# weihaoysgs/ssvio

Measured on AMD Instinct MI355X. Metric: stereo frames/s (ORB extract + row-band match + triangulate + one local BA per frame) on 1241x376, higher is better.
Workload: dtype u8 (front-end) + f64 (BA)

## Files before the change

include/ssx_test_hooks.h:

```cpp
#ifndef SSX_TEST_HOOKS_H
#define SSX_TEST_HOOKS_H
#include "ssx.h"

#ifdef __cplusplus
extern "C" {
#endif

SSX_API int32_t ssx_ba_window_selftest(uint32_t seed, int32_t steps);

SSX_API int64_t ssx_debug_kernel_dynamic_lds(const char* kernel);
SSX_API void ssx_debug_set_dense_slabs(int32_t mode);

SSX_API void ssx_debug_set_trial_finish(int32_t mode);

SSX_API double ssx_ba_debug_prepare_seconds(const ssx_ba_problem* prob, int32_t reps);

SSX_API int32_t ssx_ba_debug_upload_format(const ssx_ba_problem* prob);

SSX_API uint64_t ssx_ba_debug_prepare_digest(const ssx_ba_problem* prob, int32_t threads);

typedef struct ssx_orb_plan_info {
  int32_t status, n_buffers;
  uint64_t digest[3];
  uint64_t arena_bytes, buf_off[32], buf_bytes[32];
  int32_t nlevels, out_cap;
  int32_t lvl_rows[8], lvl_cols[8], feat[8], lvl_cell0[9], gauss_tile0[9];
  char error[256];
} ssx_orb_plan_info;
SSX_API ssx_status ssx_orb_debug_plan(int32_t rows, int32_t cols, int32_t images, const ssx_orb_params* prm, int32_t has_mask,
                                      int32_t detect_only, int32_t unchecked, ssx_orb_plan_info* out);


SSX_API ssx_status ssx_ba_linearize(ssx_ctx* ctx, const ssx_ba_problem* prob, double huber_delta, int32_t jac_mode,
                            double* Hpp, double* bp, double* Hll, double* bl, double* Hpl, double* err,
                            double* chi2);

SSX_API ssx_status ssx_orb_stage_level(ssx_ctx* ctx, int32_t image, int32_t level, int32_t blurred,
                                       uint8_t* out, int32_t out_cap, int32_t* rows, int32_t* cols);
SSX_API ssx_status ssx_orb_stage_candidates(ssx_ctx* ctx, int32_t image, int32_t level, int32_t cap,
                                            ssx_keypoint* out, int32_t* n);

SSX_API ssx_status ssx_lk_stage_level(ssx_ctx* ctx, int32_t which, int32_t level, uint8_t* out, int32_t out_cap,
                                      int32_t* rows, int32_t* cols);
SSX_API ssx_status ssx_lk_stage_deriv(ssx_ctx* ctx, int32_t level, int16_t* out, int32_t out_cap, int32_t* rows,
                                      int32_t* cols);

enum { SSX_LK_STAGED = 0, SSX_LK_ARENA = 1, SSX_LK_EACH = 2, SSX_LK_IN_PLACE = 3 };
enum { SSX_LK_K_PYRAMID = 0, SSX_LK_K_PAD_LEVEL0 = 1, SSX_LK_K_PYR_DOWN = 2, SSX_LK_K_SCHARR = 3, SSX_LK_K_TRACK = 4 };
enum { SSX_LK_SPANS = 7, SSX_LK_MAX_LAUNCHES = 32, SSX_LK_MAX_INFO_JOBS = 256 };
typedef struct ssx_lk_call_info {
  int32_t status;
  char error[256];
  int32_t levels, win, pad, rows[8], cols[8], pitch[8];
  uint64_t off[8], doff[8], pyr_bytes, deriv_words;
  int32_t fused_ok, use_fused, scharr_now, intake;
  uint64_t span_off[7], span_bytes[7], in_bytes, host_end, io_bytes, arena_bytes;
  int32_t n_launches, n_jobs;
  struct { int32_t kernel, grid[3], which, level; } launch[32];
  uint8_t slot_flags[256], job_roles[256];
} ssx_lk_call_info;
typedef struct ssx_lk_job_facts {
  int32_t slot, fresh, n, prev_stride, next_stride, reserved;
  int64_t next_off;
// ... 25 lines not shown
```

ssvio_amd/csrc/orb.hip:

```cpp
#include <algorithm>
#include <cfloat>
#include <cmath>
#include <vector>

#include "ctx.hpp"
#include "orb_ws.hpp"
#include "../../include/ssx_test_hooks.h"

namespace ssxorb {

__constant__ __attribute__((aligned(16))) int8_t c_pattern[256 * 4] = {
#include "brief_pattern.inc"
};
__constant__ int c_umax[16] = {15, 15, 15, 15, 14, 14, 14, 13, 13, 12, 11, 10, 9, 8, 6, 3};
__constant__ int c_gauss[7] = {18, 34, 49, 55, 49, 34, 18};
__constant__ int c_ring_dx[16] = {0, 1, 2, 3, 3, 3, 2, 1, 0, -1, -2, -3, -3, -3, -2, -1};
__constant__ int c_ring_dy[16] = {3, 3, 2, 1, 0, -1, -2, -3, -3, -3, -2, -1, 0, 1, 2, 3};

struct ResizeQuad {
  uint32_t s0;
  uint32_t sel0, sel1;
  uint32_t pad;
  uint32_t w[4];
};
// ... 405 lines not shown

__device__ __forceinline__ bool gauss_tile_at_edge(int rows, int cols, int x0)
{
  return rows >= 8 && cols >= 8 && (x0 == 0 || x0 + GT_W + 4 > cols);
}
__device__ __forceinline__ void gauss_fix_edges(uint8_t* sIn, int cols, int x0, int t)
{
  if (t < 6 * (GT_H + 6)) {
    const int r = t / 6, k = t - 6 * r;
    const int x = k < 3 ? k - 3 : cols + k - 3;
    const int xs = k < 3 ? -x : 2 * cols - 2 - x;
    const int b = x - x0 + 4, bs = xs - x0 + 4;
    if (b >= 0 && b < GT_PITCH && bs >= 0 && bs < GT_PITCH) sIn[r * GT_PITCH + b] = sIn[r * GT_PITCH + bs];
  }
}

__global__ __launch_bounds__(256) void k_gauss7(OrbDev o)
{
  __shared__ __attribute__((aligned(16))) uint8_t sIn[(GT_H + 6) * GT_PITCH];
  __shared__ __attribute__((aligned(16))) uint32_t sRowP[(GT_H + 6) / 2 * GT_W];
  static_assert((GT_H + 6) % 2 == 0, "rows are processed in pairs");
  const int img = blockIdx.y, t = threadIdx.x;
  int level = 0;
  while (level + 1 < o.nlevels && (int)blockIdx.x >= o.gauss_tile0[level + 1]) ++level;
  const int grp = blockIdx.x - o.gauss_tile0[level];
  const int rows = o.lvl_rows[level], cols = o.lvl_cols[level], pitch = o.lvl_pitch[level];
  const int tiles_x = (cols + GT_W - 1) / GT_W;
  const int run = o.gauss_run;
  const int groups_x = (tiles_x + run - 1) / run;
  const int ty_ = grp / groups_x, tx0 = (grp - ty_ * groups_x) * run;
  const int tx1 = min(tx0 + run, tiles_x);
  const int y0 = ty_ * GT_H;
  const uint8_t* src = o.pyr + (size_t)img * o.pyr_bytes + o.lvl_off[level];
  uint8_t* dst = o.blur + (size_t)img * o.pyr_bytes + o.lvl_off[level];
  constexpr int NDW = GT_PITCH / 4;
  uint32_t ld[GT_NLD];
  gauss_load_tile(src, rows, cols, pitch, tx0 * GT_W, y0, t, ld);
  uint32_t outv[4];
  const int og = t & 31, orq = t >> 5;
  auto store_tile = [&](int x0s) {
    const int x = x0s + 4 * og;
#pragma unroll
    for (int j = 0; j < 4; ++j) {
      const int y = y0 + 4 * orq + j;
      if (y < rows && x < pitch) *reinterpret_cast<uint32_t*>(dst + (size_t)y * pitch + x) = outv[j];
    }
  };
#pragma unroll 1
  for (int tx_ = tx0; tx_ < tx1; ++tx_) {
  const int x0 = tx_ * GT_W;
  if (tx_ > tx0) __syncthreads();
#pragma unroll
  for (int k = 0; k < GT_NLD; ++k) {
    const int i = t + 256 * k;
    if (i < (GT_H + 6) * NDW) reinterpret_cast<uint32_t*>(sIn)[i] = ld[k];
  }
  if (tx_ + 1 < tx1) gauss_load_tile(src, rows, cols, pitch, x0 + GT_W, y0, t, ld);
  if (tx_ > tx0) store_tile(x0 - GT_W);
  if (gauss_tile_at_edge(rows, cols, x0)) {
    __syncthreads();
    gauss_fix_edges(sIn, cols, x0, t);
  }
  __syncthreads();
  constexpr uint32_t W_LO = 18u | (34u << 8) | (49u << 16) | (55u << 24);
  constexpr uint32_t W_HI = 49u | (34u << 8) | (18u << 16);
  for (int i = t; i < (GT_H + 6) / 2 * (GT_W / 4); i += 256) {
    const int rp = i / (GT_W / 4), g = i - rp * (GT_W / 4);
    uint32_t sum[2][4];
#pragma unroll
    for (int h = 0; h < 2; ++h) {
      const uint32_t* rowdw = reinterpret_cast<const uint32_t*>(sIn + (2 * rp + h) * GT_PITCH) + g;
      const uint32_t d0 = rowdw[0], d1 = rowdw[1], d2 = rowdw[2];
      sum[h][0] = __builtin_amdgcn_udot4(__builtin_amdgcn_alignbyte(d1, d0, 1), W_LO, 0u, false);
      sum[h][0] = __builtin_amdgcn_udot4(__builtin_amdgcn_alignbyte(d2, d1, 1), W_HI, sum[h][0], false);
      sum[h][1] = __builtin_amdgcn_udot4(__builtin_amdgcn_alignbyte(d1, d0, 2), W_LO, 0u, false);
      sum[h][1] = __builtin_amdgcn_udot4(__builtin_amdgcn_alignbyte(d2, d1, 2), W_HI, sum[h][1], false);
      sum[h][2] = __builtin_amdgcn_udot4(__builtin_amdgcn_alignbyte(d1, d0, 3), W_LO, 0u, false);
      sum[h][2] = __builtin_amdgcn_udot4(__builtin_amdgcn_alignbyte(d2, d1, 3), W_HI, sum[h][2], false);
      sum[h][3] = __builtin_amdgcn_udot4(d1, W_LO, 0u, false);
// ... 68 lines not shown
    base += r * pitch + 4 * d;
  }
  const int step = (64 / NDW) * pitch + 4 * (64 % NDW), wrap = pitch - 4 * NDW;
#pragma unroll
  for (int i0 = 0; i0 < ROWS * NDW; i0 += 64) {
    const int i = i0 + lane;
    v[i0 / 64] = i < ROWS * NDW ? *reinterpret_cast<const uint32_t*>(base) : 0u;
    d += 64 % NDW;
    base += step;
    if (d >= NDW) { d -= NDW; base += wrap; }
  }
  return x0 - ax;
}
template <int ROWS, int NDW>
__device__ __forceinline__ void write_patch(uint32_t* sp, const uint32_t (&v)[(ROWS * NDW + 63) / 64], int lane)
{
#pragma unroll
  for (int i0 = 0; i0 < ROWS * NDW; i0 += 64)
    if (i0 + lane < ROWS * NDW) sp[i0 + lane] = v[i0 / 64];
}
template <int ROWS, int NDW, int MUL, int SH>
__device__ __forceinline__ int stage_patch(uint32_t* sp, const uint8_t* src, int pitch, int x0, int y0, int lane)
{
  uint32_t v[(ROWS * NDW + 63) / 64];
  const int off = load_patch<ROWS, NDW, MUL, SH>(v, src, pitch, x0, y0, lane);
  write_patch<ROWS, NDW>(sp, v, lane);
  return off;
}

constexpr int OP_NDW = 9;
constexpr int BP = 37, BR = 18;
constexpr int BP_NDW = 10;
constexpr int PATCH_LDS_DW = 31 * OP_NDW + BP * BP_NDW;

struct IcTables { uint2 w[16][8]; };

__device__ __forceinline__ void ic_tables_init(IcTables& tb)
{
  const int t = threadIdx.x;
  if (t < 128) {
    const int av = t >> 3, k = t & 7, dmax = c_umax[av];
    uint32_t w1 = 0, w0 = 0;
#pragma unroll
    for (int j = 0; j < 4; ++j) {
      const int u = 4 * k + j - 15;
      if (u >= -dmax && u <= dmax) { w1 |= (uint32_t)(u + 15) << (8 * j); w0 |= 1u << (8 * j); }
    }
    tb.w[av][k] = make_uint2(w1, w0);
  }
}

__device__ __forceinline__ float ic_angle(const uint32_t* sp, int off, int lane, const IcTables& tb)
{
  int m10 = 0, m01 = 0;
  if (lane < 62) {
    const int row = lane >> 1, half = lane & 1;
    const int v = row - 15, av = v < 0 ? -v : v;
    const uint32_t* rp = sp + row * OP_NDW + 4 * half;
    uint32_t d[5];
#pragma unroll
    for (int k = 0; k < 5; ++k) d[k] = rp[k];
    uint32_t s1 = 0, s0 = 0;
#pragma unroll
    for (int k = 0; k < 4; ++k) {
      const uint32_t px = __builtin_amdgcn_alignbyte(d[k + 1], d[k], off);
      const uint2 w = tb.w[av][4 * half + k];
// ... 67 lines not shown
  __shared__ IcTables sIc;
  ic_tables_init(sIc);
  __syncthreads();
  const int img = blockIdx.y;
  const int wave = __builtin_amdgcn_readfirstlane(threadIdx.x >> 6), lane = threadIdx.x & 63;
  const int slot0 = (blockIdx.x * 4 + wave) * OB_KPW;
  int cnt[MAX_LEVELS];
#pragma unroll
  for (int l = 0; l < MAX_LEVELS; ++l) cnt[l] = l < o.nlevels ? o.sel_count[img * o.nlevels + l] : 0;
  uint32_t pat[4];
  brief_pattern_of_lane(lane, pat);
  int lvl_of[OB_KPW];
  uint32_t cand[OB_KPW];
  bool ok[OB_KPW];
#pragma unroll
  for (int j = 0; j < OB_KPW; ++j) {
    const int slot = slot0 + j;
    int level = 0, base = 0, n = cnt[0];
#pragma unroll
    for (int l = 1; l < MAX_LEVELS; ++l) {
      const bool next = l < o.nlevels && level == l - 1 && slot >= base + n;
      base = next ? base + n : base;
      level = next ? l : level;
      n = next ? cnt[l] : n;
    }
    const int k = slot - base;
    ok[j] = k < n && slot < o.out_cap;
    if (k < n && slot >= o.out_cap && lane == 0) atomicOr(&o.status[img], 4);
    lvl_of[j] = level;
    cand[j] = ok[j] ? o.sel[(size_t)(img * o.nlevels + level) * SEL_CAP + k] : 0u;
  }
  uint32_t* sp = sPatch[wave];
  const int minB = EDGE_THRESHOLD - 3;
  uint32_t vr[(31 * OP_NDW + 63) / 64], vb[(BP * BP_NDW + 63) / 64];
  int off_o = 0, off_b = 0;
  auto request = [&](int j) {
    const uint32_t p = cand[j];
    const int cx = (int)(p & 0xFFF) + minB, cy = (int)((p >> 12) & 0xFFF) + minB;
    const size_t lvl = (size_t)img * o.pyr_bytes + o.lvl_off[lvl_of[j]];
    const int pitch = o.lvl_pitch[lvl_of[j]];
    off_o = load_patch<31, OP_NDW, 57, 9>(vr, o.pyr + lvl, pitch, cx - 15, cy - 15, lane);
    off_b = load_patch<BP, BP_NDW, 205, 11>(vb, o.blur + lvl, pitch, cx - BR, cy - BR, lane);
  };
  unsigned long long word_prev = 0;
  float angle_prev = 0.f;
  auto store = [&](int j) {
    const int slot = slot0 + j, level = lvl_of[j];
    const uint32_t p = cand[j];
    if (lane < 4) reinterpret_cast<unsigned long long*>(o.out_desc + ((size_t)img * o.out_cap + slot) * 32)[lane] = word_prev;
    if (lane == 0) {
      ssx_keypoint kp;
      const float sc = o.scale[level];
      kp.x = (float)((int)(p & 0xFFF) + minB); kp.y = (float)((int)((p >> 12) & 0xFFF) + minB);
      if (level != 0) { kp.x *= sc; kp.y *= sc; }
      kp.size = (float)(int)(31 * sc);
      kp.angle = angle_prev;
      kp.response = (float)(p >> 24);
      kp.octave = level;
      kp.class_id = -1;
      reinterpret_cast<ssx_keypoint*>(o.out_kps)[(size_t)img * o.out_cap + slot] = kp;
    }
  };
  if (!ok[0]) return;
  request(0);
#pragma unroll
  for (int j = 0; j < OB_KPW; ++j) {
    if (!ok[j]) break;
    const int oo = off_o, ob = off_b;
    write_patch<31, OP_NDW>(sp, vr, lane);
    write_patch<BP, BP_NDW>(sp + 31 * OP_NDW, vb, lane);
    if (j + 1 < OB_KPW && ok[j + 1]) request(j + 1);
    if (j > 0) store(j - 1);
    __builtin_amdgcn_fence(__ATOMIC_RELEASE, "workgroup");
    __builtin_amdgcn_wave_barrier();
    const float angle = ic_angle(sp, oo, lane, sIc);
    unsigned long long words[4];
    brief_words(reinterpret_cast<const uint8_t*>(sp + 31 * OP_NDW), ob, angle, pat, words);
    word_prev = (lane & 2) ? ((lane & 1) ? words[3] : words[2]) : ((lane & 1) ? words[1] : words[0]);
    angle_prev = angle;
    __builtin_amdgcn_wave_barrier();
    if (j + 1 == OB_KPW || !ok[j + 1]) store(j);
  }
}

struct DescribeAt {
  const ssx_keypoint* in;
  ssx_keypoint* out;
  uint8_t* desc;
  uint8_t* keep;
  int n_in;
};

__global__ __launch_bounds__(256) void k_describe_at(OrbDev o, DescribeAt a)
{
  __shared__ uint32_t sPatch[4][PATCH_LDS_DW];
  __shared__ IcTables sIc;
  ic_tables_init(sIc);
  const int wave = __builtin_amdgcn_readfirstlane(threadIdx.x >> 6), lane = threadIdx.x & 63;
  const int k = blockIdx.x * 4 + wave;
  bool active = k < a.n_in;
  ssx_keypoint kp{};
  int level = 0, cx = 0, cy = 0;
  float sc = 1.f;
  if (active) {
    kp = a.in[k];
    level = kp.octave;
    active = level >= 0 && level < o.nlevels;
  }
  if (active) {
    sc = o.scale[level];
    kp.x = kp.x / sc; kp.y = kp.y / sc;
    const int rows = o.lvl_rows[level], cols = o.lvl_cols[level];
    active = (kp.y - EDGE_THRESHOLD >= 0 && kp.y + EDGE_THRESHOLD < rows && kp.x - EDGE_THRESHOLD >= 0 &&
              kp.x + EDGE_THRESHOLD < cols);
    cx = __float2int_rn(kp.x); cy = __float2int_rn(kp.y);
  }
  const uint8_t* lvl = o.pyr + o.lvl_off[level];
  const int pitch = o.lvl_pitch[level];
  if (active) active = fast_score(lvl + (size_t)cy * pitch + cx, pitch, min(max(o.min_th, 0), 255)) >= 0;
  uint32_t* sp = sPatch[wave];
  int off_o = 0;
  if (active) off_o = stage_patch<31, OP_NDW, 57, 9>(sp, lvl, pitch, cx - 15, cy - 15, lane);
  __syncthreads();
  float angle = 0.f;
  if (active) angle = ic_angle(sp, off_o, lane, sIc);
  float ox = kp.x * sc, oy = kp.y * sc;
  const float dx = ox / sc, dy = oy / sc;
  const int bx = __float2int_rn(dx), by = __float2int_rn(dy);
  const uint8_t* blur = o.blur + o.lvl_off[level];
  int off_b = 0;
  if (active) off_b = stage_patch<BP, BP_NDW, 205, 11>(sp + 31 * OP_NDW, blur, pitch, bx - BR, by - BR, lane);
  __syncthreads();
  if (!active) { if (k < a.n_in && lane == 0) a.keep[k] = 0; return; }
  unsigned long long words[4];
  uint32_t pat[4];
  brief_pattern_of_lane(lane, pat);
  brief_words(reinterpret_cast<const uint8_t*>(sp + 31 * OP_NDW), off_b, angle, pat, words);
  if (lane < 4) reinterpret_cast<unsigned long long*>(a.desc + (size_t)k * 32)[lane] = words[lane];
  if (lane == 0) {
    ssx_keypoint okp = kp;
    okp.x = ox; okp.y = oy;
    okp.angle = angle;
    okp.size = 31 * sc;
    a.out[k] = okp;
    a.keep[k] = 1;
  }
}

__global__ __launch_bounds__(256) void k_finalize_detect(OrbDev o)
{
  const int img = blockIdx.y;
  const int il = img * o.nlevels;
  const int n = o.sel_count[il];
  const int k = blockIdx.x * 256 + threadIdx.x;
  if (k >= n) return;
  if (k >= o.out_cap) { atomicOr(&o.status[img], 4); return; }
  const uint32_t p = o.sel[(size_t)il * SEL_CAP + k];
  const int minB = EDGE_THRESHOLD - 3;
  ssx_keypoint kp;
  kp.x = (float)(p & 0xFFF) + (float)minB;
  kp.y = (float)((p >> 12) & 0xFFF) + (float)minB;
  kp.size = 7.f; kp.angle = -1.f; kp.response = (float)(p >> 24); kp.octave = 0; kp.class_id = -1;
  reinterpret_cast<ssx_keypoint*>(o.out_kps)[(size_t)img * o.out_cap + k] = kp;
}
// ... 63 lines not shown
  OrbDev dev{};
  std::vector<Cell> cells; std::vector<ResizeQuad> xtab; std::vector<uint2> ytab;
  size_t off[ARENA_BUFS], bytes[ARENA_BUFS], arena_bytes = 0;
};
template <class... A> ssx_status plan_fail(char* err, ssx_status st, const char* fmt, A... a) { snprintf(err, PLAN_ERR, fmt, a...); return st; }

ssx_status check_key(const PlanKey& k, const ssx_orb_params& prm, char* err)
{
  if (k.rows <= 2 * EDGE_THRESHOLD || k.cols <= 2 * EDGE_THRESHOLD || k.rows > 4000 || k.cols > 4000)
    return plan_fail(err, SSX_ERR_INVALID_ARG, "ssx_orb: image %dx%d outside the supported range (40..4000 per side)", k.cols, k.rows);
  if (k.nlevels < 1 || k.nlevels > MAX_LEVELS || !(k.scale_factor > 1.0f) || k.nfeatures < 1 || k.nfeatures > SEL_CAP - 8 || k.I < 1)
    return plan_fail(err, SSX_ERR_INVALID_ARG, "ssx_orb: unsupported parameters (nlevels=%d scale=%g nfeatures=%d)", prm.nlevels, (double)k.scale_factor, k.nfeatures);
  return SSX_OK;
}

ssx_status plan_levels(const PlanKey& k, OrbPlan& p, char* err)
{
  OrbDev& d = p.dev;
  const int nlevels = d.nlevels = k.nlevels;
  d.I = k.I; d.ini_th = k.ini_th; d.min_th = k.min_th; d.has_mask = k.has_mask; d.detect_only = k.detect_only;
  float scale[MAX_LEVELS], inv[MAX_LEVELS];
  scale[0] = 1.0f;
  for (int i = 1; i < nlevels; ++i) scale[i] = scale[i - 1] * k.scale_factor;
  for (int i = 0; i < nlevels; ++i) inv[i] = 1.0f / scale[i];
  if (k.detect_only) {
    d.feat[0] = k.nfeatures;
  } else {
    const float factor = 1.0f / k.scale_factor;
    float nDesired = k.nfeatures * (1 - factor) / (1 - (float)std::pow((double)factor, (double)nlevels));
    int sum = 0;
    for (int l = 0; l < nlevels - 1; ++l) { d.feat[l] = h_round(nDesired); sum += d.feat[l]; nDesired *= factor; }
    d.feat[nlevels - 1] = std::max(k.nfeatures - sum, 0);
  }
  size_t off = 0;
  for (int l = 0; l < nlevels; ++l) {
    d.scale[l] = scale[l];
    d.lvl_cols[l] = h_round((float)k.cols * inv[l]);
    d.lvl_rows[l] = h_round((float)k.rows * inv[l]);
    d.lvl_pitch[l] = (d.lvl_cols[l] + 127) & ~127;
    d.lvl_off[l] = off;
    off += (size_t)d.lvl_pitch[l] * d.lvl_rows[l];
    if (d.feat[l] + 8 > SEL_CAP) return plan_fail(err, SSX_ERR_UNSUPPORTED, "ssx_orb: %d features on level %d exceed the octree node capacity", d.feat[l], l);
  }
  d.pyr_bytes = (off + 255) & ~size_t(255);
  return SSX_OK;
}

void plan_cells(OrbPlan& p)
{
  OrbDev& d = p.dev;
  d.out_cap = 32;
  for (int l = 0; l < d.nlevels; ++l) {
    d.lvl_cell0[l] = (int)p.cells.size();
    make_cells(d.lvl_rows[l], d.lvl_cols[l], l, p.cells);
    const int bw = d.lvl_cols[l] - 2 * (EDGE_THRESHOLD - 3), bh = d.lvl_rows[l] - 2 * (EDGE_THRESHOLD - 3);
    const int n_ini = bh > 0 ? (int)std::lround((double)bw / (double)bh) : 0;
    d.out_cap += std::max(d.feat[l] + 4, 4 * std::max(n_ini, 0) + 4);
  }
  for (int l = d.nlevels; l <= MAX_LEVELS; ++l) d.lvl_cell0[l] = (int)p.cells.size();
  d.n_cells = (int)p.cells.size();
}

ssx_status plan_octree(OrbPlan& p, char* err)
{
  OrbDev& d = p.dev;
  int maxN = 256;
  for (int l = 0; l < (d.detect_only ? 1 : d.nlevels); ++l) maxN = std::max(maxN, d.feat[l]);
  d.oct_ln = (maxN + 8 + 7) & ~7;
  d.oct_max_cells = 1;
  for (int l = 0; l < d.nlevels; ++l) d.oct_max_cells = std::max(d.oct_max_cells, d.lvl_cell0[l + 1] - d.lvl_cell0[l]);
  d.oct_global_keys = (size_t)d.lvl_rows[0] * d.lvl_cols[0] > 600000;
  d.oct_cand_cap = d.oct_global_keys ? CAND_CAP_BIG : CAND_CAP;
  const size_t key_lds = d.oct_global_keys ? 0 : 6 * (size_t)CAND_CAP;
  if (4 * (size_t)(d.oct_max_cells + 8) + key_lds > (size_t)OCT_LDS_BUDGET)
    return plan_fail(err, SSX_ERR_UNSUPPORTED, "ssx_orb: %d grid cells on one level exceed the octree workgroup's LDS", d.oct_max_cells);
  d.oct_global_tab = (size_t)OCT_NODE_BYTES * d.oct_ln + 4 * (size_t)(d.oct_max_cells + 8) + key_lds > (size_t)OCT_LDS_BUDGET;
  d.oct_stride = ((d.oct_global_keys ? 6 * (size_t)CAND_CAP_BIG : 0) + (d.oct_global_tab ? (size_t)OCT_NODE_BYTES * d.oct_ln : 0) + 255) & ~size_t(255);
// ... 38 lines not shown
        fx -= sx;
        if (sx < 0) { fx = 0; sx = 0; }
        if (sx >= scols - 1) { fx = 0; sx = scols - 1; }
        const int a0 = h_round((1.f - fx) * 2048), a1 = h_round(fx * 2048);
        const int sx1 = std::min(sx + 1, scols - 1);
        if (j == 0) rq.s0 = (uint32_t)sx;
        const int o0 = sx - (int)rq.s0, o1 = sx1 - (int)rq.s0;
        if (o1 > 7) d.rs_wide8[l] = 0;
        if (o1 > 255) return plan_fail(err, SSX_ERR_UNSUPPORTED, "ssx_orb: pyramid scale factor %g is too large for the resize tables", (double)k.scale_factor);
        rq.sel0 |= (uint32_t)o0 << (8 * j);
        rq.sel1 |= (uint32_t)o1 << (8 * j);
        rq.w[j] = (uint32_t)a0 | ((uint32_t)a1 << 16);
      }
      p.xtab.push_back(rq);
    }
    for (int dy = 0; dy < drows; ++dy) {
      float fy = (float)((dy + 0.5) * scale_y - 0.5);
      const int sy = (int)std::floor(fy);
      fy -= sy;
      const int b0 = h_round((1.f - fy) * 2048), b1 = h_round(fy * 2048);
      const int sy0 = std::min(std::max(sy, 0), srows - 1), sy1 = std::min(std::max(sy + 1, 0), srows - 1);
      p.ytab.push_back(make_uint2((uint32_t)sy0 | ((uint32_t)sy1 << 16), (uint32_t)b0 | ((uint32_t)b1 << 16)));
    }
  }
  return SSX_OK;
}

template <class F> void for_each_buffer(OrbPlan& p, F&& f)
{
  OrbDev& d = p.dev;
  const size_t I = (size_t)d.I, IL = I * d.nlevels, cells = (size_t)std::max(d.n_cells, 1);
  f(d.cells, sizeof(Cell) * std::max<size_t>(p.cells.size(), 1));
  f(d.rs_xtab, sizeof(ResizeQuad) * std::max<size_t>(p.xtab.size(), 1)); f(d.rs_ytab, sizeof(uint2) * std::max<size_t>(p.ytab.size(), 4));
  f(d.pyr, d.pyr_bytes * I); f(d.maskpyr, d.has_mask ? d.pyr_bytes * I : 256); f(d.blur, d.pyr_bytes * I);
  f(d.cell_count, sizeof(int) * I * cells); f(d.cell_cand, sizeof(uint32_t) * I * cells * CELL_CAP);
  f(d.oct, std::max<size_t>(d.oct_stride * IL, 256)); f(d.lvl_ncand, sizeof(int) * IL); f(d.sel_count, sizeof(int) * IL);
  f(d.sel, sizeof(uint32_t) * IL * SEL_CAP); f(d.sel_angle, sizeof(float) * IL * SEL_CAP);
  f(d.status, sizeof(int) * I); f(d.out_kps, sizeof(ssx_keypoint) * I * d.out_cap); f(d.out_desc, (size_t)32 * I * d.out_cap); f(d.out_n, sizeof(int) * I);
}

void plan_arena(OrbPlan& p)
{
  Layout lay;
  int n = 0;
  for_each_buffer(p, [&](auto*&, size_t bytes) { p.bytes[n] = bytes; p.off[n++] = lay.take(bytes); });
  p.arena_bytes = lay.off;
}

ssx_status build_plan(const PlanKey& k, OrbPlan& p, char* err)
{
  ssx_status st = plan_levels(k, p, err);
  if (st != SSX_OK) return st;
  plan_cells(p);
  if ((st = plan_octree(p, err)) != SSX_OK) return st;
  plan_tiles(p);
  if ((st = plan_resize(k, p, err)) != SSX_OK) return st;
  for (const Cell& c : p.cells)
    if (c.w > ROI_MAX || c.h > ROI_MAX) return plan_fail(err, SSX_ERR_UNSUPPORTED, "ssx_orb: grid cell %dx%d exceeds the %d-px LDS tile", c.w, c.h, ROI_MAX);
  plan_arena(p);
  return SSX_OK;
}

#ifndef SSX_NO_TEST_HOOKS
void plan_digest(const OrbDev& d, const size_t* offs, int n_offs, const std::vector<Cell>& cells, const std::vector<ResizeQuad>& xtab,
                 const std::vector<uint2>& ytab, uint64_t out[3])
{
  uint64_t h = 0;
  auto eat = [&](const void* p, size_t n) { const uint8_t* b = (const uint8_t*)p; for (size_t i = 0; i < n; ++i) { h ^= b[i]; h *= 1099511628211ull; } };
#define SSX_EAT(x) eat(&d.x, sizeof(d.x))
  h = 1469598103934665603ull;
  SSX_EAT(I); SSX_EAT(nlevels); SSX_EAT(lvl_rows); SSX_EAT(lvl_cols); SSX_EAT(lvl_pitch); SSX_EAT(lvl_off); SSX_EAT(pyr_bytes); SSX_EAT(scale); SSX_EAT(feat);
  SSX_EAT(lvl_cell0); SSX_EAT(n_cells); SSX_EAT(ini_th); SSX_EAT(min_th); SSX_EAT(has_mask); SSX_EAT(detect_only); SSX_EAT(out_cap); SSX_EAT(fast_tile_bytes);
  SSX_EAT(fast_lds_per_wave); SSX_EAT(gauss_tile0); SSX_EAT(gauss_run); SSX_EAT(rs_xoff); SSX_EAT(rs_yoff); SSX_EAT(rs_wide8); SSX_EAT(oct_stride);
  SSX_EAT(oct_max_cells); SSX_EAT(oct_cand_cap); SSX_EAT(oct_global_keys); SSX_EAT(oct_ln); SSX_EAT(oct_global_tab);
#undef SSX_EAT
  out[0] = h;
  h = 1469598103934665603ull;
  eat(offs, sizeof(size_t) * n_offs);
  out[1] = h;
  h = 1469598103934665603ull;
  const size_t n[3] = {cells.size(), xtab.size(), ytab.size()};
  eat(n, sizeof(n)); eat(cells.data(), sizeof(Cell) * n[0]); eat(xtab.data(), sizeof(ResizeQuad) * n[1]); eat(ytab.data(), sizeof(uint2) * n[2]);
  out[2] = h;
}
#endif

}

ssx_status plan(ssx_ctx* ctx, int rows, int cols, int I, const ssx_orb_params& prm, bool has_mask, bool detect_only)
{
  OrbWorkspace* ws = get_ws(ctx);
  const PlanKey key{rows, cols, I, detect_only ? 1 : prm.nlevels, prm.nfeatures, prm.ini_th_fast, prm.min_th_fast, has_mask, detect_only, prm.scale_factor};
  char err[PLAN_ERR] = {0};
  ssx_status st = check_key(key, prm, err);
  if (st == SSX_OK && ws->planned && ws->key == key) return SSX_OK;
  OrbPlan p;
  if (st == SSX_OK) st = build_plan(key, p, err);
  if (st != SSX_OK) { ctx->set_error("%s", err); return st; }
  SSX_HIP_TRY(ctx, hipSetDevice(ctx->device));
  SSX_HIP_TRY(ctx, hipStreamSynchronize(ctx->stream));
  SSX_HIP_TRY(ctx, ws->arena.reserve(p.arena_bytes));
  int n = 0;
  for_each_buffer(p, [&](auto*& ptr, size_t) { wire(ptr, ws->arena.as<char>(), p.off[n++]); });
  const OrbDev& d = p.dev;
// ... 355 lines not shown
ssx_status ssx_orb_describe_at(ssx_ctx* ctx, const uint8_t* img, int32_t stride, int32_t rows, int32_t cols,
                               const ssx_orb_params* prm, const ssx_keypoint* kps_in, int32_t n_in, ssx_keypoint* kps_out,
                               uint8_t* desc_out, int32_t* n)
{
  if (!ctx || !prm || !n) return SSX_ERR_INVALID_ARG;
  *n = 0;
  if (!img || rows <= 0 || cols <= 0 || n_in <= 0 || !kps_in) return SSX_OK;
  if (stride < cols || !kps_out || !desc_out) {
    ctx->set_error("ssx_orb_describe_at: stride smaller than the image width or no output arrays");
    return SSX_ERR_INVALID_ARG;
  }
  Described d;
  ssx_status st = describe_enqueue(ctx, img, stride, rows, cols, *prm, kps_in, n_in, 0, &d);
  if (st != SSX_OK) return st;
  OrbWorkspace* ws = get_ws(ctx);
  auto host = [&](const void* dev) { return ws->stage.as<char>() + ((const char*)dev - d.base); };
  SSX_HIP_TRY(ctx, hipMemcpyAsync(host(d.kps), d.kps, d.total - ((const char*)d.kps - d.base), hipMemcpyDeviceToHost, ctx->stream));
  SSX_HIP_TRY(ctx, hipStreamSynchronize(ctx->stream));
  const ssx_keypoint* ok = (const ssx_keypoint*)host(d.kps);
  const uint8_t* od = (const uint8_t*)host(d.desc);
  const uint8_t* keep = (const uint8_t*)host(d.keep);
  int m = 0;
  for (int i = 0; i < n_in; ++i) {
    if (!keep[i]) continue;
    if (kps_out) kps_out[m] = ok[i];
    if (desc_out) memcpy(desc_out + (size_t)32 * m, od + (size_t)32 * i, 32);
    ++m;
  }
  *n = m;
  return SSX_OK;
}

#ifndef SSX_NO_TEST_HOOKS
ssx_status ssx_orb_debug_plan(int32_t rows, int32_t cols, int32_t images, const ssx_orb_params* prm, int32_t has_mask, int32_t detect_only,
                              int32_t unchecked, ssx_orb_plan_info* out)
{
  if (!prm || !out) return SSX_ERR_INVALID_ARG;
  *out = ssx_orb_plan_info{};
  const PlanKey key{rows, cols, images, detect_only ? 1 : prm->nlevels, prm->nfeatures, prm->ini_th_fast, prm->min_th_fast, has_mask != 0, detect_only != 0, prm->scale_factor};
  static_assert(sizeof(out->error) == PLAN_ERR, "ssx_orb_plan_info::error holds the plan's error text");
  OrbPlan p;
  ssx_status st = unchecked && key.nlevels >= 1 && key.nlevels <= MAX_LEVELS ? SSX_OK : check_key(key, *prm, out->error);
  if (st == SSX_OK) st = build_plan(key, p, out->error);
  out->status = st;
  if (st != SSX_OK) return st;
  const OrbDev& d = p.dev;
  size_t offs[ARENA_BUFS + 1];
  for (int b = 0; b < ARENA_BUFS; ++b) { out->buf_off[b] = offs[b] = p.off[b]; out->buf_bytes[b] = p.bytes[b]; }
  out->n_buffers = ARENA_BUFS;
  out->arena_bytes = offs[ARENA_BUFS] = p.arena_bytes;
  out->nlevels = d.nlevels; out->out_cap = d.out_cap;
  memcpy(out->lvl_rows, d.lvl_rows, sizeof(d.lvl_rows)); memcpy(out->lvl_cols, d.lvl_cols, sizeof(d.lvl_cols)); memcpy(out->feat, d.feat, sizeof(d.feat));
  memcpy(out->lvl_cell0, d.lvl_cell0, sizeof(d.lvl_cell0)); memcpy(out->gauss_tile0, d.gauss_tile0, sizeof(d.gauss_tile0));
  plan_digest(d, offs, ARENA_BUFS + 1, p.cells, p.xtab, p.ytab, out->digest);
  return SSX_OK;
}

ssx_status ssx_orb_stage_level(ssx_ctx* ctx, int32_t image, int32_t level, int32_t blurred, uint8_t* out,
                               int32_t out_cap, int32_t* rows, int32_t* cols)
{
  if (!ctx || !ctx->orb || !ctx->orb->planned) return SSX_ERR_INVALID_ARG;
  const OrbDev& d = ctx->orb->dev;
  if (image < 0 || image >= d.I || level < 0 || level >= d.nlevels) return SSX_ERR_INVALID_ARG;
  const int r = d.lvl_rows[level], c = d.lvl_cols[level];
  if (rows) *rows = r;
  if (cols) *cols = c;
  if (!out) return SSX_OK;
  if (out_cap < r * c) return SSX_ERR_CAPACITY;
  const uint8_t* src = (blurred ? d.blur : d.pyr) + (size_t)image * d.pyr_bytes + d.lvl_off[level];
  SSX_HIP_TRY(ctx, hipMemcpy2DAsync(out, c, src, d.lvl_pitch[level], c, r, hipMemcpyDeviceToHost, ctx->stream));
  SSX_HIP_TRY(ctx, hipStreamSynchronize(ctx->stream));
  return SSX_OK;
}

ssx_status ssx_orb_stage_candidates(ssx_ctx* ctx, int32_t image, int32_t level, int32_t cap, ssx_keypoint* out,
                                    int32_t* n)
{
  if (!ctx || !ctx->orb || !ctx->orb->planned || !n) return SSX_ERR_INVALID_ARG;
  const OrbDev& d = ctx->orb->dev;
  if (image < 0 || image >= d.I || level < 0 || level >= d.nlevels) return SSX_ERR_INVALID_ARG;
  const int c0 = d.lvl_cell0[level], c1 = d.lvl_cell0[level + 1];
  const int nc = c1 - c0;
  std::vector<int> cnt(std::max(nc, 1));
  std::vector<uint32_t> cand((size_t)std::max(nc, 1) * CELL_CAP);
  if (nc > 0) {
    SSX_HIP_TRY(ctx, hipMemcpyAsync(cnt.data(), d.cell_count + (size_t)image * d.n_cells + c0, sizeof(int) * nc, hipMemcpyDeviceToHost, ctx->stream));
    SSX_HIP_TRY(ctx, hipMemcpyAsync(cand.data(), d.cell_cand + ((size_t)image * d.n_cells + c0) * CELL_CAP,
                                    sizeof(uint32_t) * (size_t)nc * CELL_CAP, hipMemcpyDeviceToHost, ctx->stream));
    SSX_HIP_TRY(ctx, hipStreamSynchronize(ctx->stream));
  }
  int m = 0;
  for (int c = 0; c < nc; ++c)
    for (int k = 0; k < cnt[c]; ++k, ++m) {
      if (m >= cap || !out) continue;
      const uint32_t p = cand[(size_t)c * CELL_CAP + k];
      ssx_keypoint kp;
      kp.x = (float)(p & 0xFFF); kp.y = (float)((p >> 12) & 0xFFF); kp.size = 7.f; kp.angle = -1.f;
      kp.response = (float)(p >> 24); kp.octave = 0; kp.class_id = -1;
      out[m] = kp;
    }
  *n = m;
  return (out && m > cap) ? SSX_ERR_CAPACITY : SSX_OK;
// ... 6 lines not shown
```

ssvio_amd/csrc/orb_ws.hpp:

```cpp
#pragma once
#include <hip/hip_runtime.h>

#include <cstdint>
#include <vector>

#include "ctx.hpp"

namespace ssxorb {

constexpr int MAX_LEVELS = 8;
constexpr int CELL_CAP = 256;
constexpr int CAND_CAP = 16384;
constexpr int CAND_CAP_BIG = 65536;
constexpr int SEL_CAP = 4096;
constexpr int EDGE_THRESHOLD = 19;
constexpr int OCT_THREADS = 1024;

struct Cell {
  int16_t x0, y0;
  int16_t w, h;
  int16_t ox, oy;
  int16_t level, pad;
};

constexpr int OCT_NODE_BYTES = 50;
constexpr int OCT_LDS_BUDGET = 158 * 1024;

struct ResizeQuad;

struct OrbDev {
  int I;
  int nlevels;
  int lvl_rows[MAX_LEVELS], lvl_cols[MAX_LEVELS], lvl_pitch[MAX_LEVELS];
  size_t lvl_off[MAX_LEVELS];
  size_t pyr_bytes;
  float scale[MAX_LEVELS];
  int feat[MAX_LEVELS];
  int lvl_cell0[MAX_LEVELS + 1];
  int n_cells;
  int ini_th, min_th;
  int has_mask;
  int detect_only;
  int out_cap;
  int fast_tile_bytes;
  int fast_lds_per_wave;
  int gauss_tile0[MAX_LEVELS + 1];
  int gauss_run;
  int rs_xoff[MAX_LEVELS], rs_yoff[MAX_LEVELS];
  int rs_wide8[MAX_LEVELS];
  const Cell* cells;
  const ResizeQuad* rs_xtab;
  const uint2* rs_ytab;
  uint8_t* pyr;
  uint8_t* maskpyr;
  uint8_t* blur;
  int* cell_count;
  uint32_t* cell_cand;
  uint8_t* oct;
  size_t oct_stride;
  int oct_max_cells;
  int oct_cand_cap;
  int oct_global_keys;
  int oct_ln;
  int oct_global_tab;
  int* lvl_ncand;
  int* sel_count;
  uint32_t* sel;
  float* sel_angle;
// ... 74 lines not shown
```

Before: 17450.

## Store blurred pyramid in 16x8 blocked layout for patch gathers

```diff
diff --git a/include/ssx_test_hooks.h b/include/ssx_test_hooks.h
--- a/include/ssx_test_hooks.h
+++ b/include/ssx_test_hooks.h
@@ -29,6 +29,8 @@
 } ssx_orb_plan_info;
 SSX_API ssx_status ssx_orb_debug_plan(int32_t rows, int32_t cols, int32_t images, const ssx_orb_params* prm, int32_t has_mask,
                                       int32_t detect_only, int32_t unchecked, ssx_orb_plan_info* out);
+
+SSX_API ssx_status ssx_orb_debug_blur_map(int32_t pitch, int32_t rows, uint32_t* out, uint64_t* level_bytes);
 
 
 SSX_API ssx_status ssx_ba_linearize(ssx_ctx* ctx, const ssx_ba_problem* prob, double huber_delta, int32_t jac_mode,
diff --git a/ssvio_amd/csrc/orb.hip b/ssvio_amd/csrc/orb.hip
--- a/ssvio_amd/csrc/orb.hip
+++ b/ssvio_amd/csrc/orb.hip
@@ -461,19 +461,31 @@
   const int tx1 = min(tx0 + run, tiles_x);
   const int y0 = ty_ * GT_H;
   const uint8_t* src = o.pyr + (size_t)img * o.pyr_bytes + o.lvl_off[level];
-  uint8_t* dst = o.blur + (size_t)img * o.pyr_bytes + o.lvl_off[level];
+  uint8_t* dst = o.blur + (size_t)img * o.blur_bytes + o.blur_off[level];
   constexpr int NDW = GT_PITCH / 4;
   uint32_t ld[GT_NLD];
   gauss_load_tile(src, rows, cols, pitch, tx0 * GT_W, y0, t, ld);
   uint32_t outv[4];
   const int og = t & 31, orq = t >> 5;
+  const int o_row = y0 + 4 * orq + ((og >> 2) & 3);
+  const uint32_t o_blk = (uint32_t)blur_byte(4 * (og & 3) + 4 * BLK_W * (og >> 4), o_row, pitch);
   auto store_tile = [&](int x0s) {
-    const int x = x0s + 4 * og;
-#pragma unroll
-    for (int j = 0; j < 4; ++j) {
-      const int y = y0 + 4 * orq + j;
-      if (y < rows && x < pitch) *reinterpret_cast<uint32_t*>(dst + (size_t)y * pitch + x) = outv[j];
-    }
+    const bool hi4 = og & 4, hi8 = og & 8;
+#pragma unroll
+    for (int p = 0; p < 4; p += 2) {
+      const uint32_t got = (uint32_t)__builtin_amdgcn_ds_swizzle((int)(hi4 ? outv[p] : outv[p + 1]), (4 << 10) | 0x1F);
+      if (hi4) outv[p] = got; else outv[p + 1] = got;
+    }
+#pragma unroll
+    for (int p = 0; p < 2; ++p) {
+      const uint32_t got = (uint32_t)__builtin_amdgcn_ds_swizzle((int)(hi8 ? outv[p] : outv[p + 2]), (8 << 10) | 0x1F);
+      if (hi8) outv[p] = got; else outv[p + 2] = got;
+    }
+    uint8_t* p = dst + o_blk + (x0s >> 4) * BLK_BYTES;
+    const int x = x0s + 4 * (og & 3) + 4 * BLK_W * (og >> 4);
+#pragma unroll
+    for (int j = 0; j < 4; ++j)
+      if (o_row < rows && x + BLK_W * j < pitch) *reinterpret_cast<uint32_t*>(p + j * BLK_BYTES) = outv[j];
   };
 #pragma unroll 1
   for (int tx_ = tx0; tx_ < tx1; ++tx_) {
@@ -608,6 +620,45 @@
 constexpr int BP = 37, BR = 18;
 constexpr int BP_NDW = 10;
 constexpr int PATCH_LDS_DW = 31 * OP_NDW + BP * BP_NDW;
+
+constexpr int BP_ROUNDS = (BP * BP_NDW + 63) / 64;
+static_assert(BP_ROUNDS % 2 == 0 && BP_NDW > 2 * (BLK_W / 4) && BP_NDW <= 3 * (BLK_W / 4) && 4 * BP < 512 / 3, "load_patch_blocked: block columns of a patch, g / wb");
+__device__ __forceinline__ int load_patch_blocked(uint32_t (&v)[BP_ROUNDS], uint32_t (&dst)[BP_ROUNDS / 2], const uint8_t* src, int pitch, int x0, int y0, int lane)
+{
+  const int ax = x0 & ~3;
+  const int yb = y0 & 7, a4 = (ax >> 2) & 3, w0 = 4 - a4;
+  const int bpr = pitch >> 4;
+  const uint8_t* base = src + ((size_t)(y0 >> 3) * bpr + (ax >> 4)) * BLK_BYTES;
+  const int c1 = BP * w0, c2 = c1 + 4 * BP, c3 = c2 + 4 * BP;
+  const int w2 = min(4, BP_NDW - 4 - w0), w3 = BP_NDW - 8 - w0;
+  auto recip = [](int w) { return (int)((0x008000AB01000200ull >> (16 * ((w - 1) & 3))) & 0xFFFFu); };
+  const int m0 = recip(w0), m2 = recip(w2), m3 = recip(w3);
+#pragma unroll
+  for (int n = 0; n < BP_ROUNDS; ++n) {
+    const int s1 = c1 - 64 * n, s2 = c2 - 64 * n, s3 = c3 - 64 * n;
+    const bool b1 = lane >= s1, b2 = lane >= s2, b3 = lane >= s3;
+    const int b = (int)b1 + (int)b2 + (int)b3;
+    const int start = b3 ? s3 : b2 ? s2 : b1 ? s1 : -64 * n;
+    const int ds = b1 ? w0 + 4 * (b - 1) : 0;
+    const int wb = b3 ? w3 : b2 ? w2 : b1 ? 4 : w0;
+    const int g = lane - start;
+    const int r = (g * (b3 ? m3 : b2 ? m2 : b1 ? 128 : m0)) >> 9;
+    const int dd = g - r * wb;
+    const int gr = yb + r;
+    const uint32_t off = (uint32_t)(((gr >> 3) * bpr + b) * BLK_BYTES + (gr & 7) * BLK_W + 4 * ((b1 ? 0 : a4) + dd));
+    v[n] = lane < BP * BP_NDW - 64 * n ? *reinterpret_cast<const uint32_t*>(base + off) : 0u;
+    const uint32_t at = (uint32_t)(r * BP_NDW + ds + dd);
+    if (n & 1) dst[n / 2] |= at << 16; else dst[n / 2] = at;
+    __builtin_amdgcn_sched_barrier(0);
+  }
+  return x0 - ax;
+}
+__device__ __forceinline__ void write_patch_blocked(uint32_t* sp, const uint32_t (&v)[BP_ROUNDS], const uint32_t (&dst)[BP_ROUNDS / 2], int lane)
+{
+#pragma unroll
+  for (int n = 0; n < BP_ROUNDS; ++n)
+    if (64 * n + lane < BP * BP_NDW) sp[(dst[n / 2] >> (16 * (n & 1))) & 0xFFFFu] = v[n];
+}
 
 struct IcTables { uint2 w[16][8]; };
 
@@ -741,7 +792,7 @@
   }
   uint32_t* sp = sPatch[wave];
   const int minB = EDGE_THRESHOLD - 3;
-  uint32_t vr[(31 * OP_NDW + 63) / 64], vb[(BP * BP_NDW + 63) / 64];
+  uint32_t vr[(31 * OP_NDW + 63) / 64], vb[BP_ROUNDS], vb_at[BP_ROUNDS / 2];
   int off_o = 0, off_b = 0;
   auto request = [&](int j) {
     const uint32_t p = cand[j];
@@ -749,7 +800,7 @@
     const size_t lvl = (size_t)img * o.pyr_bytes + o.lvl_off[lvl_of[j]];
     const int pitch = o.lvl_pitch[lvl_of[j]];
     off_o = load_patch<31, OP_NDW, 57, 9>(vr, o.pyr + lvl, pitch, cx - 15, cy - 15, lane);
-    off_b = load_patch<BP, BP_NDW, 205, 11>(vb, o.blur + lvl, pitch, cx - BR, cy - BR, lane);
+    off_b = load_patch_blocked(vb, vb_at, o.blur + (size_t)img * o.blur_bytes + o.blur_off[lvl_of[j]], pitch, cx - BR, cy - BR, lane);
   };
   unsigned long long word_prev = 0;
   float angle_prev = 0.f;
@@ -777,7 +828,7 @@
     if (!ok[j]) break;
     const int oo = off_o, ob = off_b;
     write_patch<31, OP_NDW>(sp, vr, lane);
-    write_patch<BP, BP_NDW>(sp + 31 * OP_NDW, vb, lane);
+    write_patch_blocked(sp + 31 * OP_NDW, vb, vb_at, lane);
     if (j + 1 < OB_KPW && ok[j + 1]) request(j + 1);
     if (j > 0) store(j - 1);
     __builtin_amdgcn_fence(__ATOMIC_RELEASE, "workgroup");
@@ -836,9 +887,13 @@
   float ox = kp.x * sc, oy = kp.y * sc;
   const float dx = ox / sc, dy = oy / sc;
   const int bx = __float2int_rn(dx), by = __float2int_rn(dy);
-  const uint8_t* blur = o.blur + o.lvl_off[level];
+  const uint8_t* blur = o.blur + o.blur_off[level];
   int off_b = 0;
-  if (active) off_b = stage_patch<BP, BP_NDW, 205, 11>(sp + 31 * OP_NDW, blur, pitch, bx - BR, by - BR, lane);
+  if (active) {
+    uint32_t vb[BP_ROUNDS], vb_at[BP_ROUNDS / 2];
+    off_b = load_patch_blocked(vb, vb_at, blur, pitch, bx - BR, by - BR, lane);
+    write_patch_blocked(sp + 31 * OP_NDW, vb, vb_at, lane);
+  }
   __syncthreads();
   if (!active) { if (k < a.n_in && lane == 0) a.keep[k] = 0; return; }
   unsigned long long words[4];
@@ -968,7 +1023,7 @@
     for (int l = 0; l < nlevels - 1; ++l) { d.feat[l] = h_round(nDesired); sum += d.feat[l]; nDesired *= factor; }
     d.feat[nlevels - 1] = std::max(k.nfeatures - sum, 0);
   }
-  size_t off = 0;
+  size_t off = 0, boff = 0;
   for (int l = 0; l < nlevels; ++l) {
     d.scale[l] = scale[l];
     d.lvl_cols[l] = h_round((float)k.cols * inv[l]);
@@ -976,9 +1031,12 @@
     d.lvl_pitch[l] = (d.lvl_cols[l] + 127) & ~127;
     d.lvl_off[l] = off;
     off += (size_t)d.lvl_pitch[l] * d.lvl_rows[l];
+    d.blur_off[l] = boff;
+    boff += (size_t)d.lvl_pitch[l] * blur_rows(d.lvl_rows[l]);
     if (d.feat[l] + 8 > SEL_CAP) return plan_fail(err, SSX_ERR_UNSUPPORTED, "ssx_orb: %d features on level %d exceed the octree node capacity", d.feat[l], l);
   }
   d.pyr_bytes = (off + 255) & ~size_t(255);
+  d.blur_bytes = (boff + 255) & ~size_t(255);
   return SSX_OK;
 }
 
@@ -1083,7 +1141,7 @@
   const size_t I = (size_t)d.I, IL = I * d.nlevels, cells = (size_t)std::max(d.n_cells, 1);
   f(d.cells, sizeof(Cell) * std::max<size_t>(p.cells.size(), 1));
   f(d.rs_xtab, sizeof(ResizeQuad) * std::max<size_t>(p.xtab.size(), 1)); f(d.rs_ytab, sizeof(uint2) * std::max<size_t>(p.ytab.size(), 4));
-  f(d.pyr, d.pyr_bytes * I); f(d.maskpyr, d.has_mask ? d.pyr_bytes * I : 256); f(d.blur, d.pyr_bytes * I);
+  f(d.pyr, d.pyr_bytes * I); f(d.maskpyr, d.has_mask ? d.pyr_bytes * I : 256); f(d.blur, d.blur_bytes * I);
   f(d.cell_count, sizeof(int) * I * cells); f(d.cell_cand, sizeof(uint32_t) * I * cells * CELL_CAP);
   f(d.oct, std::max<size_t>(d.oct_stride * IL, 256)); f(d.lvl_ncand, sizeof(int) * IL); f(d.sel_count, sizeof(int) * IL);
   f(d.sel, sizeof(uint32_t) * IL * SEL_CAP); f(d.sel_angle, sizeof(float) * IL * SEL_CAP);
@@ -1120,7 +1178,7 @@
   auto eat = [&](const void* p, size_t n) { const uint8_t* b = (const uint8_t*)p; for (size_t i = 0; i < n; ++i) { h ^= b[i]; h *= 1099511628211ull; } };
 #define SSX_EAT(x) eat(&d.x, sizeof(d.x))
   h = 1469598103934665603ull;
-  SSX_EAT(I); SSX_EAT(nlevels); SSX_EAT(lvl_rows); SSX_EAT(lvl_cols); SSX_EAT(lvl_pitch); SSX_EAT(lvl_off); SSX_EAT(pyr_bytes); SSX_EAT(scale); SSX_EAT(feat);
+  SSX_EAT(I); SSX_EAT(nlevels); SSX_EAT(lvl_rows); SSX_EAT(lvl_cols); SSX_EAT(lvl_pitch); SSX_EAT(lvl_off); SSX_EAT(pyr_bytes); SSX_EAT(blur_off); SSX_EAT(blur_bytes); SSX_EAT(scale); SSX_EAT(feat);
   SSX_EAT(lvl_cell0); SSX_EAT(n_cells); SSX_EAT(ini_th); SSX_EAT(min_th); SSX_EAT(has_mask); SSX_EAT(detect_only); SSX_EAT(out_cap); SSX_EAT(fast_tile_bytes);
   SSX_EAT(fast_lds_per_wave); SSX_EAT(gauss_tile0); SSX_EAT(gauss_run); SSX_EAT(rs_xoff); SSX_EAT(rs_yoff); SSX_EAT(rs_wide8); SSX_EAT(oct_stride);
   SSX_EAT(oct_max_cells); SSX_EAT(oct_cand_cap); SSX_EAT(oct_global_keys); SSX_EAT(oct_ln); SSX_EAT(oct_global_tab);
@@ -1542,6 +1600,16 @@
 }
 
 #ifndef SSX_NO_TEST_HOOKS
+ssx_status ssx_orb_debug_blur_map(int32_t pitch, int32_t rows, uint32_t* out, uint64_t* level_bytes)
+{
+  if (pitch <= 0 || pitch % 128 != 0 || rows <= 0 || (size_t)pitch * blur_rows(rows) > 0xFFFFFFFFull) return SSX_ERR_INVALID_ARG;
+  if (level_bytes) *level_bytes = (uint64_t)pitch * blur_rows(rows);
+  if (out)
+    for (int y = 0; y < blur_rows(rows); ++y)
+      for (int x = 0; x < pitch; ++x) out[(size_t)y * pitch + x] = (uint32_t)blur_byte(x, y, pitch);
+  return SSX_OK;
+}
+
 ssx_status ssx_orb_debug_plan(int32_t rows, int32_t cols, int32_t images, const ssx_orb_params* prm, int32_t has_mask, int32_t detect_only,
                               int32_t unchecked, ssx_orb_plan_info* out)
 {
@@ -1577,7 +1645,16 @@
   if (cols) *cols = c;
   if (!out) return SSX_OK;
   if (out_cap < r * c) return SSX_ERR_CAPACITY;
-  const uint8_t* src = (blurred ? d.blur : d.pyr) + (size_t)image * d.pyr_bytes + d.lvl_off[level];
+  if (blurred) {
+    const int pitch = d.lvl_pitch[level];
+    std::vector<uint8_t> blk((size_t)pitch * blur_rows(r));
+    SSX_HIP_TRY(ctx, hipMemcpyAsync(blk.data(), d.blur + (size_t)image * d.blur_bytes + d.blur_off[level], blk.size(), hipMemcpyDeviceToHost, ctx->stream));
+    SSX_HIP_TRY(ctx, hipStreamSynchronize(ctx->stream));
+    for (int y = 0; y < r; ++y)
+      for (int x = 0; x < c; ++x) out[(size_t)y * c + x] = blk[blur_byte(x, y, pitch)];
+    return SSX_OK;
+  }
+  const uint8_t* src = d.pyr + (size_t)image * d.pyr_bytes + d.lvl_off[level];
   SSX_HIP_TRY(ctx, hipMemcpy2DAsync(out, c, src, d.lvl_pitch[level], c, r, hipMemcpyDeviceToHost, ctx->stream));
   SSX_HIP_TRY(ctx, hipStreamSynchronize(ctx->stream));
   return SSX_OK;
diff --git a/ssvio_amd/csrc/orb_ws.hpp b/ssvio_amd/csrc/orb_ws.hpp
--- a/ssvio_amd/csrc/orb_ws.hpp
+++ b/ssvio_amd/csrc/orb_ws.hpp
@@ -28,12 +28,21 @@
 
 struct ResizeQuad;
 
+constexpr int BLK_W = 16, BLK_H = 8, BLK_BYTES = BLK_W * BLK_H;
+__host__ __device__ inline int blur_rows(int rows) { return (rows + BLK_H - 1) & ~(BLK_H - 1); }
+__host__ __device__ inline size_t blur_byte(int x, int y, int pitch)
+{
+  return ((size_t)(y >> 3) * (pitch >> 4) + (x >> 4)) * BLK_BYTES + (y & 7) * BLK_W + (x & 15);
+}
+
 struct OrbDev {
   int I;
   int nlevels;
   int lvl_rows[MAX_LEVELS], lvl_cols[MAX_LEVELS], lvl_pitch[MAX_LEVELS];
   size_t lvl_off[MAX_LEVELS];
   size_t pyr_bytes;
+  size_t blur_off[MAX_LEVELS];
+  size_t blur_bytes;
   float scale[MAX_LEVELS];
   int feat[MAX_LEVELS];
   int lvl_cell0[MAX_LEVELS + 1];
```

Result: no change. 17570 (median of 4 runs) (+0.7%).
